# khanhha/temporal_inverse_kinematics

Measured on AMD Instinct MI355X. Metric: IK frames/sec (COCO-17->SMPLx pose), higher is better.
Workload: dtype f32 via bf16x3 (x = 3 bf16 planes, 6 MFMA products, fp32 accumulate; fp32 exponent range); 1 GPU; ST-GCN IK forward, batch=1024x64-frame x COCO-17 windows per GPU -> (B,4,66) SMPL-X pose; global_batch=1024, window_frames=64, out_frames=4, parallelism=single

## Files before the change

### include/tik.h

```cpp
#ifndef TIK_H
#define TIK_H

#include <stdint.h>

#ifdef __cplusplus
extern "C" {
#endif

#define TIK_OK 0
#define TIK_E_INVALID (-1)
#define TIK_E_HIP (-2)
#define TIK_E_MISSING (-3)
#define TIK_E_NOMEM (-4)

typedef struct tik_model* tik_model_t;
typedef struct tik_fk* tik_fk_t;

typedef struct {
    const char* name;
    const float* data;
    int ndim;
    int64_t shape[4];
} tik_tensor;

const char* tik_last_error(void);
const char* tik_version(void);
int tik_debug_check_guards(void);
int tik_debug_alloc_fill(void);
int tik_debug_checksums(char* buf, int len);

int tik_model_create(const tik_tensor* tensors, int n_tensors, tik_model_t* out);
int tik_model_destroy(tik_model_t m);
int tik_model_out_frames(tik_model_t m, int T);
int tik_model_reserve(tik_model_t m, int N, int T);
int tik_ik_forward(tik_model_t m, const float* x, int N, int T, float* poses, void* stream);
int tik_backbone_forward(tik_model_t m, const float* x, int N, int T, float* feat, void* stream);

#define TIK_PREC_F32 0
#define TIK_PREC_BF16X3 2
int tik_model_set_precision(tik_model_t m, int prec);
int tik_model_get_precision(tik_model_t m);

int tik_model_profile(tik_model_t m, int max_launches);
int tik_model_profile_count(tik_model_t m);
int tik_model_profile_read(tik_model_t m, int i, char* label, int label_len, float* ms, double* flops,
                           double* bytes);

typedef struct tik_block* tik_block_t;
int tik_block_create(const tik_tensor* tensors, int n_tensors, int in_channels, int out_channels,
                     int stride, int residual, const float* A_eff_host, int V, tik_block_t* out);
int tik_block_destroy(tik_block_t b);
int tik_stgcn_block_fwd(tik_block_t b, const float* x, int N, int T, float* out, void* stream);
int tik_block_set_precision(tik_block_t b, int prec);

int tik_gconv_fwd(const float* x, int N, int Cin, int T, int V, const float* A, int K,
                  const float* W, const float* b, int Cout, int t_kernel, int t_stride,
                  int t_padding, int t_dilation, float* out, void* stream);

int tik_aa_to_rotmat(const float* aa, int n, float* R, void* stream);

int tik_window_gather(const float* seq, int F, int V, int idx0, int n_idx, int h, int root_a,
                      int root_b, int relative, float* windows, void* stream);

int tik_moveai_to_coco(const float* joints, int F, int J, const int* map17_host, float* out, void* stream);

typedef struct tik_stream* tik_stream_t;
int tik_stream_create(tik_model_t model, int win_size, int use_graph, tik_stream_t* out);
int tik_stream_destroy(tik_stream_t s);
int tik_stream_reset(tik_stream_t s);
int tik_stream_push(tik_stream_t s, const float* frame_host, float* pose_host);
int tik_stream_path(tik_stream_t s);
int tik_debug_stream_trace(tik_stream_t s, long long* out, int cap);
int tik_debug_stream_inject_error(tik_stream_t s);
int tik_debug_stream_set_count(tik_stream_t s, int count);

int tik_rotate_root_z(float* poses, int F, int ld, double angle, void* stream);
int tik_train_windows(const float* joints, int n_joints, const float* poses, int pose_ld, const int* item_start,
                      const int* item_len, const int* item_idx, const int* item_uid, int B, int h,
                      const int* coco_map, const float* sigma, int relative, int add_noise, unsigned long long seed,
                      float* windows, float* target, void* stream);

typedef struct tik_trainer* tik_trainer_t;
// ... 35 lines not shown
```

### temporal_inverse_kinematics_amd/_lib.py

```python
from __future__ import annotations

import ctypes
import os
from typing import Dict, Iterable, Tuple

import numpy as np
import torch

LIB_PATH = os.environ.get("TIK_LIB") or os.path.join(os.path.dirname(os.path.abspath(__file__)), "libtik.so")

TIK_OK, TIK_E_INVALID, TIK_E_HIP, TIK_E_MISSING, TIK_E_NOMEM = 0, -1, -2, -3, -4


class TikTensor(ctypes.Structure):
    _fields_ = [("name", ctypes.c_char_p), ("data", ctypes.POINTER(ctypes.c_float)),
                ("ndim", ctypes.c_int), ("shape", ctypes.c_int64 * 4)]


_P = ctypes.c_void_p
_I = ctypes.c_int
_F = ctypes.POINTER(ctypes.c_float)

SIGNATURES: Dict[str, Tuple[object, Tuple]] = {
    "tik_last_error": (ctypes.c_char_p, ()),
    "tik_version": (ctypes.c_char_p, ()),
    "tik_debug_check_guards": (_I, ()),
    "tik_debug_alloc_fill": (_I, ()),
    "tik_debug_checksums": (_I, (ctypes.c_char_p, _I)),
    "tik_model_create": (_I, (ctypes.POINTER(TikTensor), _I, ctypes.POINTER(_P))),
    "tik_model_destroy": (_I, (_P,)),
    "tik_model_out_frames": (_I, (_P, _I)),
    "tik_model_reserve": (_I, (_P, _I, _I)),
    "tik_ik_forward": (_I, (_P, _P, _I, _I, _P, _P)),
    "tik_backbone_forward": (_I, (_P, _P, _I, _I, _P, _P)),
    "tik_model_set_precision": (_I, (_P, _I)),
    "tik_model_get_precision": (_I, (_P,)),
    "tik_block_set_precision": (_I, (_P, _I)),
    "tik_fk_set_precision": (_I, (_P, _I)),
    "tik_model_profile": (_I, (_P, _I)),
    "tik_model_profile_count": (_I, (_P,)),
    "tik_model_profile_read": (_I, (_P, _I, ctypes.c_char_p, _I, ctypes.POINTER(ctypes.c_float),
                                    ctypes.POINTER(ctypes.c_double), ctypes.POINTER(ctypes.c_double))),
    "tik_block_create": (_I, (ctypes.POINTER(TikTensor), _I, _I, _I, _I, _I, _F, _I, ctypes.POINTER(_P))),
    "tik_block_destroy": (_I, (_P,)),
    "tik_stgcn_block_fwd": (_I, (_P, _P, _I, _I, _P, _P)),
    "tik_gconv_fwd": (_I, (_P, _I, _I, _I, _I, _P, _I, _P, _P, _I, _I, _I, _I, _I, _P, _P)),
    "tik_aa_to_rotmat": (_I, (_P, _I, _P, _P)),
    "tik_window_gather": (_I, (_P, _I, _I, _I, _I, _I, _I, _I, _I, _P, _P)),
    "tik_moveai_to_coco": (_I, (_P, _I, _I, ctypes.POINTER(ctypes.c_int), _P, _P)),
    "tik_stream_create": (_I, (_P, _I, _I, ctypes.POINTER(_P))),
    "tik_stream_destroy": (_I, (_P,)),
    "tik_stream_reset": (_I, (_P,)),
    "tik_stream_push": (_I, (_P, _F, _F)),
    "tik_stream_path": (_I, (_P,)),
    "tik_rotate_root_z": (_I, (_P, _I, _I, ctypes.c_double, _P)),
    "tik_train_windows": (_I, (_P, _I, _P, _I, _P, _P, _P, _P, _I, _I, _P, _P, _I, _I, ctypes.c_ulonglong, _P, _P, _P)),
    "tik_debug_stream_trace": (_I, (_P, ctypes.POINTER(ctypes.c_longlong), _I)),
    "tik_debug_stream_inject_error": (_I, (_P,)),
    "tik_debug_stream_set_count": (_I, (_P, _I)),
    "tik_fk_create": (_I, (ctypes.POINTER(TikTensor), _I, _I, ctypes.POINTER(_P))),
    "tik_fk_destroy": (_I, (_P,)),
    "tik_fk_num_joints": (_I, (_P,)),
    "tik_fk_num_verts": (_I, (_P,)),
    "tik_fk_reserve": (_I, (_P, _I)),
    "tik_fk_forward": (_I, (_P, _P, _P, _P, _P, _I, _P, _P, _P)),
    "tik_fk_joints": (_I, (_P, _P, _P, _P, _P, _I, ctypes.POINTER(_I), _I, _P, _P)),
    "tik_fk_workspace_bytes": (ctypes.c_longlong, (_P,)),
    "tik_fk_profile": (_I, (_P, _I)),
    "tik_fk_profile_count": (_I, (_P,)),
    "tik_fk_profile_read": (_I, (_P, _I, ctypes.c_char_p, _I, ctypes.POINTER(ctypes.c_float),
                                 ctypes.POINTER(ctypes.c_double), ctypes.POINTER(ctypes.c_double))),
    "tik_trainer_create": (_I, (ctypes.POINTER(TikTensor), _I, ctypes.c_float, ctypes.POINTER(_P))),
    "tik_trainer_destroy": (_I, (_P,)),
    "tik_trainer_step": (_I, (_P, _P, _I, _I, _P, _P, ctypes.c_ulonglong, _P, _P)),
    "tik_trainer_out_frames": (_I, (_P, _I)),
    "tik_trainer_count": (_I, (_P,)),
    "tik_trainer_tensor": (_I, (_P, _I, ctypes.c_char_p, _I, ctypes.POINTER(ctypes.c_int64), ctypes.POINTER(_I),
                                ctypes.POINTER(_I))),
    "tik_trainer_read": (_I, (_P, _I, _I, _P, _P)),
    "tik_trainer_steps": (ctypes.c_longlong, (_P,)),
    "tik_trainer_debug": (_I, (_P, _I, _I, _P, ctypes.c_longlong, _P)),
# ... 85 lines not shown
```

### temporal_inverse_kinematics_amd/csrc/debug.cpp

```cpp
#include <hip/hip_runtime.h>

#include <algorithm>
#include <map>
#include <mutex>

#include "misc.h"
#include "model.h"

namespace tik_host {
std::atomic<int> g_alloc_fill{-1};
thread_local Profiler* g_prof = nullptr;

bool guard_mode() {
    static const bool on = getenv("TIK_GUARD") && getenv("TIK_GUARD")[0] == '1';
    return on;
}
static std::mutex g_guard_mu;
static std::map<void*, size_t> g_guard_bufs;
void guard_register(void* base, size_t bytes) {
    std::lock_guard<std::mutex> l(g_guard_mu);
    g_guard_bufs[base] = bytes;
}
void guard_unregister(void* base) {
    std::lock_guard<std::mutex> l(g_guard_mu);
// ... 97 lines not shown
}
using namespace tik_host;

extern "C" {

int tik_debug_checksums(char* buf, int len) {
    if (!checksum_mode()) return fail(TIK_E_INVALID, "TIK_CHECKSUM is not set");
    const int n = (int)g_cks.size();
    if (buf && len > 0) {
        strncpy(buf, g_cks.c_str(), len - 1);
        buf[len - 1] = 0;
    }
    g_cks.clear();
    return n;
}

int tik_debug_check_guards(void) {
    if (!guard_mode()) return fail(TIK_E_INVALID, "TIK_GUARD=1 is not set");
    HIP_TRY(hipDeviceSynchronize());
    std::lock_guard<std::mutex> l(g_guard_mu);
    std::vector<unsigned char> h(GUARD_BYTES);
    int bad = 0;
    std::string rep;
    for (const auto& kv : g_guard_bufs) {
        const char* base = static_cast<const char*>(kv.first);
        for (int side = 0; side < 2; ++side) {
            const char* gp = side == 0 ? base : base + GUARD_BYTES + kv.second;
            HIP_TRY(hipMemcpy(h.data(), gp, GUARD_BYTES, hipMemcpyDeviceToHost));
            size_t first = GUARD_BYTES, last = 0, cnt = 0;
            bool clean = true;
            for (size_t i = 0; i < GUARD_BYTES && clean; i += 8) {
                unsigned long long w;
                memcpy(&w, h.data() + i, 8);
                clean = w == 0xA5A5A5A5A5A5A5A5ull;
            }
            for (size_t i = 0; i < GUARD_BYTES && !clean; ++i)
                if (h[i] != 0xA5) { first = std::min(first, i); last = i; ++cnt; }
            if (cnt) {
                ++bad;
                char b[256];
                snprintf(b, sizeof(b), "[buf %p payload %zu B: %s guard, %zu bytes changed at +%zu..+%zu] ", (const void*)(base + GUARD_BYTES),
                         kv.second, side == 0 ? "front" : "back", cnt, first, last);
                rep += b;
                HIP_TRY(hipMemset(const_cast<char*>(gp), 0xA5, GUARD_BYTES));
            }
        }
    }
    g_err = rep;
    return bad;
}

int tik_debug_alloc_fill(void) { return g_alloc_fill.load(); }

}
```

### temporal_inverse_kinematics_amd/csrc/forward.cpp

```cpp
#include <hip/hip_runtime.h>

#include <algorithm>

#include "misc.h"
#include "model.h"
#include "xtws.h"

using namespace tik_host;

namespace tik_host {

static tik::Seg mkseg(const float* src, const float* w, const SplitW3& s3, int cin, int ld, int kt, int stride, int pad,
                      int tin, int ldw) {
    tik::Seg s{src, w, cin, ld, kt, stride, pad, tin, ldw};
    s.cin8 = s3.cin8; s.ldw8 = s3.ldw8;
    for (int i = 0; i < 3; ++i) s.wb[i] = s3.p[i].p;
    return s;
}

int Layer::forward(const float* x, int ld, int N, int tin, float* z, float* out, hipStream_t st, int prec,
                   float* part) const {
    const int to = tout(tin, stride);
    tik::CgemmArgs g{};
    g.M = N * tin * V; g.Nc = cout; g.V = V; g.tout = tin;
    g.seg[0] = mkseg(x, wg.p, s3g, cinp, ld, 1, 1, 0, tin, cinp);
    g.nseg = 1;
    g.bias = bias2.p; g.out = z; g.ldo = cout; g.amix = amix.p; g.act = tik::ACT_RELU;
    g.mix_sparse = mix_sparse ? 1 : 0;
    const double px_in = (double)N * tin * V, px_out = (double)N * to * V;
    {
        const std::string lab = "G272x64.L" + std::to_string(index);
        ProfScope p(lab.c_str(), gcn_work(px_in, cin, cout, V), st);
        HIP_TRY(tik::launch_cgemm(g, tik::CFG_G272x64, st, prec));
    }

    tik::CgemmArgs t{};
    t.M = N * to * V; t.Nc = cout; t.V = V; t.tout = to;
    t.seg[0] = mkseg(z, wt.p, s3t, cout, cout, TK, stride, 1, tin, TK * cout);
    t.nseg = 1;
    if (res == RES_CONV) {
        t.seg[1] = mkseg(x, wr.p, s3r, cinp, ld, 1, stride, 0, tin, cinp);
        t.nseg = 2;
    } else if (res == RES_IDEN) {
        t.resid = x; t.ldr = ld;
    }
    t.bias = biasT.p; t.out = out; t.ldo = cout; t.act = tik::ACT_RELU;
    const bool big = cout >= 128;
    const int cfg = big ? tik::CFG_T128x128 : (prec == tik::PREC_F32 ? tik::CFG_T256x64 : tik::CFG_T128x64);
    const std::string lab = std::string(big ? "T128x128.L" : (cfg == tik::CFG_T256x64 ? "T256x64.L" : "T128x64.L")) +
                            std::to_string(index);
    if (part) {
        t.ksplit = tik::splitk_for(t, cfg == tik::CFG_T256x64 ? 256 : 128, big ? 128 : 64,
                                   prec == tik::PREC_F32 ? 16 : 32, 64);
        t.partial = part;
    }
    ProfScope p(lab.c_str(), tcn_work(px_in, px_out, cin, cout, res), st);
    HIP_TRY(tik::launch_cgemm(t, cfg, st, prec));
    return TIK_OK;
}

int Layer::spatial_x(const float* x, int ld, int N, int tin, float* z, hipStream_t st, int ncu, const RawInput* raw) const {
    const long long rin = (long long)N * tin * V;
    if (raw) {
        ProfScope p("G0f_raw.L0", gcn_work((double)rin, cin, cout, V, GCN_RAW0), st);
        HIP_TRY(tik::launch_gcn0_f32(raw->kp, (int)rin, V, cin, raw->bn_sc, raw->bn_sh, wg.p, cinp, bias2.p, amix.p, mix_sparse ? 1 : 0,
                                     cout, z, cout, raw->xb4, st));
    } else if (xgw_path()) {
        tik::XGraphArgs g{};
        g.nframes = N * tin; g.x = x; g.ldx = ld; g.cin = cin; g.cout = cout; g.wp = xgw.p;
        g.bias2 = bias2.p; g.amix = amix.p; g.mix_sparse = mix_sparse ? 1 : 0; g.out = z; g.ldo = cout;
        g.nts = 1; g.trash = xtrash;
        const std::string lab = "XGW.L" + std::to_string(index);
        ProfScope p(lab.c_str(), gcn_work((double)rin, cin, cout, V), st);
        p.out(z, (size_t)rin * cout * 4);
        HIP_TRY(launch_xgraph_traced(g, ncu, st, lab.c_str()));
    } else {
        tik::XArgs g{};
        g.M = (int)rin; g.Nc = cout; g.V = V; g.tout = tin;
        g.seg[0] = tik::XSeg{x, ld, cin, 1, 1, 0, tin, rin};
        g.nseg = 1; g.wp = xg.p; g.ksteps = xg_ks;
        g.bias = bias2.p; g.amix = amix.p; g.mix_sparse = mix_sparse ? 1 : 0; g.out = z; g.ldo = cout; g.act = tik::ACT_RELU;
        g.nw = 4; g.nts = 1;
        const std::string lab = std::string(xg_bn == 128 ? "XG128.L" : "XG64.L") + std::to_string(index);
        ProfScope p(lab.c_str(), gcn_work((double)rin, cin, cout, V), st);
        p.out(z, (size_t)rin * cout * 4);
        HIP_TRY(launch_xgemm_traced(g, xg_bn, tik::EPI_GRAPH, st, lab.c_str()));
    }
    return TIK_OK;
}

int Layer::temporal_x(const float* x, int ld, int N, int tin, const float* z, float* out, hipStream_t st, int ncu,
                      const RawInput* raw, const FusedNext* fg) const {
    const int to = tout(tin, stride);
    const long long rin = (long long)N * tin * V, rout = (long long)N * to * V;
    const double px_in = (double)rin, px_out = (double)rout;
    if (xtws_path(raw != nullptr, ld, tin)) {
        tik::XTConvArgs c{};
        c.M = (int)rout; c.T = tin; c.z = z; c.ldz = cout; c.x = x; c.ldx = ld; c.wp = xtw.p; c.bias = biasT.p;
        c.out = out; c.ldo = cout; c.nts = 1; c.trash = xtrash;
        Work w = tcn_work(px_in, px_out, cin, cout, RES_IDEN);
        if (fg) {
            const Layer& gn = *fg->layer;
            c.wg = gn.xgw.p; c.bias2 = gn.bias2.p; c.amix = gn.amix.p; c.mix_sparse = gn.mix_sparse ? 1 : 0;
            c.zout = fg->zn; c.ldzo = gn.cout;
            w = w + gcn_work(px_out, gn.cin, gn.cout, V, GCN_FUSED);
        }
        const std::string lab = (fg ? "XTWG.L" : "XTW.L") + std::to_string(index);
        ProfScope p(lab.c_str(), w, st);
        p.out(out, (size_t)rout * cout * 4);
        HIP_TRY(tik::launch_xtws(c, ncu, st));
        return TIK_OK;
    }
    tik::XArgs t{};
    t.M = (int)rout; t.Nc = cout; t.V = V; t.tout = to;
    t.seg[0] = tik::XSeg{z, cout, cout, TK, stride, 1, tin, rin};
    t.nseg = 1;
    if (raw) {
        t.rx = raw->xb4; t.rxc = cin; t.rw = wr0.p;
    } else if (res == RES_CONV) {
        t.seg[1] = tik::XSeg{x, ld, cin, 1, stride, 0, tin, rin};
        t.nseg = 2;
    } else if (res == RES_IDEN) {
        t.idn = tik::XSeg{x, ld, cin, 1, 1, 0, to, rin};
    }
    t.wp = xt.p; t.ksteps = tik::xgemm_ksteps(t);
    if (tik::xgemm_kmain(t) != xt_ks) return fail(TIK_E_INVALID, "layer %d: xgemm K steps %d != packed %d", index, tik::xgemm_kmain(t), xt_ks);
    t.bias = biasT.p; t.out = out; t.ldo = cout; t.act = tik::ACT_RELU;
    t.nw = 4; t.epi_lds = 1; t.idn_epi = 1; t.nts = 1;
// ... 264 lines not shown
```

### temporal_inverse_kinematics_amd/csrc/model.cpp

```cpp
#include <hip/hip_runtime.h>

#include <algorithm>
#include <memory>

#include "model.h"
#include "online.h"

using namespace tik_host;

namespace tik_host {

int Layer::pack(const FoldedBlock& f) {
    cin = f.cin; cinp = f.cinp; cout = f.cout; stride = f.stride; res = f.res; V = f.V; mix_sparse = f.mix_sparse;
    int rc;
    if ((rc = wg.upload(f.wg)) || (rc = bias2.upload(f.bias2)) || (rc = amix.upload(f.amix)) || (rc = wt.upload(f.wt)) ||
        (rc = biasT.upload(f.biasT)) || (rc = s3g.build(f.wg, cout, 1, cinp, cinp)) ||
        (rc = s3t.build(f.wt, cout, TK, cout, TK * cout)))
        return rc;
    if (res == RES_CONV && ((rc = wr.upload(f.wr)) || (rc = s3r.build(f.wr, cout, 1, cinp, cinp)))) return rc;
    if ((rc = wr0.upload(f.wr0))) return rc;
    const int bn = cout >= 128 ? 128 : 64;
    if (cin % 32 == 0) {
        const tik::XPackSeg g{f.wg.data(), cinp, 1, cin};
        if ((rc = xg.upload(tik::xgemm_pack(&g, 1, cout, bn)))) return rc;
        xg_bn = bn; xg_ks = cin / 32;
    }
    if (cout % 32 == 0) {
        tik::XPackSeg t[2] = {{f.wt.data(), TK * cout, TK, cout}, {f.wr.data(), cinp, 1, cin}};
        const int ns = (res == RES_CONV && cin % 32 == 0) ? 2 : 1;
        if ((rc = xt.upload(tik::xgemm_pack(t, ns, cout, bn)))) return rc;
        xt_bn = bn; xt_ks = TK * cout / 32 + (ns == 2 ? cin / 32 : 0);
    }
    if (cout == 128 && cin == 128 && stride == 1 && res == RES_IDEN)
        if ((rc = xtw.upload(tik::xblock_pack_weights(f.wt.data(), cout, TK * cout, TK, cout)))) return rc;
    if ((cout == 128 || cout == 256) && (cin == 64 || cin == 128 || cin == 256))
        if ((rc = xgw.upload(tik::xblock_pack_weights(f.wg.data(), cout, cinp, 1, cin)))) return rc;
    if (cout == 64 && stride == 1) {
        if ((rc = xbt.upload(tik::xblock_pack_weights(f.wt.data(), cout, TK * cout, TK, cout)))) return rc;
        if (cin == 64 && (rc = xbg.upload(tik::xblock_pack_weights(f.wg.data(), cout, cinp, 1, cin)))) return rc;
    }
    return TIK_OK;
}

static void apply_env(tik_model* md) {
    if (const char* e = getenv("TIK_X_CHUNK")) md->x_chunk_max = atoi(e);
    if (const char* e = getenv("TIK_XBLK")) md->xblk = e[0] != '0';
    int dev = 0, ncu = 0;
    if (hipGetDevice(&dev) == hipSuccess && hipDeviceGetAttribute(&ncu, hipDeviceAttributeMultiprocessorCount, dev) == hipSuccess && ncu > 0)
        md->ncu = ncu;
    for (auto& L : md->layers) {
        if (const char* w = getenv("TIK_XGW")) L.xgwon = (atoi(w) >> L.index) & 1;
        if (const char* w = getenv("TIK_XTWS")) L.xtwson = (atoi(w) >> L.index) & 1;
        if (const char* w = getenv("TIK_XFG")) L.xfgon = (atoi(w) >> L.index) & 1;
        L.xtrash = reinterpret_cast<float*>(md->trash.p);
    }
    if (const char* e = getenv("TIK_SPLIT")) md->split = e[0] != '0';
}

int model_reserve_ws(tik_model* m, Workspace& w, int N, int T) {
    const size_t V = m->V;
    size_t zmax = 0, amax = 0;
    int t = T;
    for (const Layer& L : m->layers) {
        zmax = std::max(zmax, (size_t)N * t * V * L.cout);
        t = Layer::tout(t, L.stride);
        amax = std::max(amax, (size_t)N * t * V * L.cout);
    }
    if (m->use_xblk()) zmax = std::max(zmax, (size_t)N * T * V * XB0_P3_FLOATS);
    size_t z2max = 0;
    t = T;
    for (size_t l = 0; l + 1 < m->layers.size(); ++l) {
        const Layer& L = m->layers[l];
        t = Layer::tout(t, L.stride);
        if (L.index > 0 && L.stride == 1 && L.fuses_gcn_of(m->layers[l + 1])) z2max = std::max(z2max, (size_t)N * t * V * m->layers[l + 1].cout);
    }
    t = T;
    for (const Layer& L : m->layers) t = Layer::tout(t, L.stride);
    int rc;
    if (z2max && (rc = w.z2.reserve(z2max))) return rc;
    if ((rc = w.xb.reserve((size_t)N * T * V * 4)) || (rc = w.z.reserve(zmax)) ||
        (rc = w.a0.reserve(amax)) || (rc = w.a1.reserve(amax)) || (rc = w.hid.reserve((size_t)N * t * m->hidden)) ||
        (rc = w.part.reserve(std::max((size_t)384 * 128 * 128, (size_t)8 * N * t * m->hidden))))
        return rc;
    return TIK_OK;
}

void model_retain(tik_model* m) { m->refs.fetch_add(1); }
int model_pose_dim(const tik_model* m) { return m->pose_dim; }
void model_release(tik_model* m) {
    if (m->refs.fetch_sub(1) == 1) delete m;
}

int model_online_fill(tik_model* m, tik::OnlineArgs& a) {
    static_assert((int)tik::ONR_ZERO == RES_ZERO && (int)tik::ONR_IDEN == RES_IDEN && (int)tik::ONR_CONV == RES_CONV, "");
    const int nl = (int)m->layers.size();
    if (m->V != 17 || m->C0 != 3 || nl > tik::ONL_MAXL) return fail(TIK_E_INVALID, "online kernel: V=17, 3 input channels, <= %d layers", tik::ONL_MAXL);
    if (m->pose_dim <= 0) return fail(TIK_E_INVALID, "online kernel: backbone-only handle (no pose_regressor weights)");
    a.nl = nl;
    for (int l = 0; l < nl; ++l) {
        const Layer& L = m->layers[l];
        if (L.cout % 16 || L.cout > tik::ONL_MAXC || L.cinp > tik::ONL_MAXC || (l > 0 && L.cinp != L.cin))
            return fail(TIK_E_INVALID, "online kernel: layer %d channels %d -> %d", l, L.cin, L.cout);
        tik::OnlineLayer& o = a.L[l];
        o.cin = L.cin; o.cinp = L.cinp; o.cout = L.cout; o.stride = L.stride; o.res = L.res;
// ... 88 lines not shown
```

### temporal_inverse_kinematics_amd/csrc/model.h

```cpp
#pragma once
#include <atomic>
#include <string>
#include <vector>

#include "cgemm.h"
#include "common.h"
#include "xblock.h"
#include "xgemm.h"
#include "xgraph.h"

namespace tik_host {

struct Work {
    double flops = 0, bytes = 0;
    Work operator+(const Work& o) const { return Work{flops + o.flops, bytes + o.bytes}; }
};
enum GcnIo {
    GCN_LAYER = 0,
    GCN_RAW0 = 1,
    GCN_FUSED = 2,
};
inline Work gcn_work(double px, int cin, int cout, int V, GcnIo io = GCN_LAYER) {
    const double x = io == GCN_FUSED ? 0.0 : px * cin;
    const double w = io == GCN_RAW0 ? 0.0 : (double)cout * cin + (double)V * (V + cout);
    return Work{2.0 * px * cin * cout + 2.0 * V * px * cout, 4.0 * (x + px * cout + w)};
}
constexpr int RES_RAW0 = 3;
inline Work tcn_work(double px_in, double px_out, int cin, int cout, int res) {
    Work w{2.0 * px_out * TK * cout * cout, 4.0 * (px_in * cout + px_out * cout + (double)TK * cout * cout)};
    if (res == RES_CONV || res == RES_RAW0) w.flops += 2.0 * px_out * cin * cout;
    if (res == RES_CONV) w.bytes += 4.0 * (px_out * cin + (double)cin * cout);
    if (res == RES_RAW0) w.bytes += 4.0 * px_out * 4;
    if (res == RES_IDEN) w.bytes += 4.0 * px_out * cout;
    return w;
}

extern thread_local Profiler* g_prof;

struct ProfScope {
    int i;
    hipStream_t st;
    const char* lab;
    const void* op = nullptr;
    size_t obytes = 0;
    void out(const void* p, size_t bytes) { op = p; obytes = bytes; }
    ProfScope(const char* label, Work w, hipStream_t s) : st(s), lab(label) {
        i = g_prof ? g_prof->begin(label, w.flops, w.bytes, s) : -1;
    }
    ~ProfScope();
};

hipError_t launch_xgemm_traced(tik::XArgs a, int bn, int epi, hipStream_t st, const char* label);
hipError_t launch_xgraph_traced(tik::XGraphArgs a, int ncu, hipStream_t st, const char* label);
hipError_t launch_xblock_traced(tik::XBlkArgs a, bool raw, int ncu, hipStream_t st, const char* label);

struct Layer;
struct RawInput {
    const float *kp, *bn_sc, *bn_sh;
    float* xb4;
};
struct FusedNext {
    const Layer* layer;
    float* zn;
};

struct Layer {
    int cin = 0, cinp = 0, cout = 0, stride = 1, res = RES_IDEN, V = 17, index = 0;
    bool mix_sparse = false;
    DevBuf wg, bias2, amix, wt, wr, biasT;
    SplitW3 s3g, s3t, s3r;
    DevBuf wr0;
    DevHBuf xg, xt;
    int xg_bn = 0, xt_bn = 0, xg_ks = 0, xt_ks = 0;
    DevHBuf xtw;
    DevHBuf xgw;
    DevHBuf xbg, xbt;
    int xgwon = 1;
    int xtwson = 1;
    int xfgon = 1;
    float* xtrash = nullptr;

    int pack(const FoldedBlock& f);

    static int tout(int tin, int s) { return (tin - 1) / s + 1; }

    bool x_ok() const { return xt.p && (xg.p || (index == 0 && wr0.p)); }
    bool xgw_path() const { return xgwon && xgw.p; }
    bool xtws_path(bool raw, int ld, int tin) const {
        return xtwson && xtw.p && !raw && res == RES_IDEN && stride == 1 && ld >= cout && ld % 4 == 0 && tin % 8 == 0;
    }
    bool fuses_gcn_of(const Layer& nx) const {
        return xfgon && xtw.p && nx.xgw_path() && nx.cin == cout && cout == 128 && nx.cout == 128;
    }
    bool xpt_path() const { return xt_bn == 64 && cout % xt_bn == 0; }

    int forward(const float* x, int ld, int N, int tin, float* z, float* out, hipStream_t st, int prec,
                float* part = nullptr) const;
    int spatial_x(const float* x, int ld, int N, int tin, float* z, hipStream_t st, int ncu,
                  const RawInput* raw) const;
    int temporal_x(const float* x, int ld, int N, int tin, const float* z, float* out, hipStream_t st, int ncu,
                   const RawInput* raw, const FusedNext* fg) const;
};

}

struct tik_model {
    int V = 17, C0 = 3, feat = 0, hidden = 0, pose_dim = 0;
    std::vector<tik_host::Layer> layers;
    tik_host::DevBuf bn_sc, bn_sh;
    tik_host::DevBuf w0, b0, w3, b3;
    tik_host::SplitW3 s30, s33;
    tik_host::DevHBuf xh0;
    static constexpr int XHEAD_KS = 4;
    int prec = 2;
    static constexpr int MAXSPLIT = 2;
    tik_host::Workspace ws[MAXSPLIT];
    hipStream_t aux[MAXSPLIT - 1] = {};
    hipEvent_t ev_fork = nullptr, ev_join[MAXSPLIT - 1] = {};
    bool split = true;
    std::atomic<int> refs{1};
    ~tik_model() {
        if (ev_fork) (void)hipEventDestroy(ev_fork);
        for (auto e : ev_join) if (e) (void)hipEventDestroy(e);
        for (auto a : aux) if (a) (void)hipStreamDestroy(a);
    }
    int x_chunk_max = 0;
    bool xblk = true;
    int ncu = 256;
    tik_host::DevHBuf trash;
    tik_host::Profiler prof;
// ... 31 lines not shown
```

### temporal_inverse_kinematics_amd/csrc/xgraph.h

```cpp
#pragma once
#include <hip/hip_runtime.h>

namespace tik {

struct XGraphArgs {
    int nframes;
    const float* x;
    int ldx;
    int cin, cout;
    const unsigned short* wp;
    const float* bias2;
    const float* amix;
    int mix_sparse;
    float* out;
    int ldo;
    int nts;
    float* trash;
    int tune;
    unsigned long long* trace;
};

bool xgraph_ok(const XGraphArgs& a);
hipError_t launch_xgraph(const XGraphArgs& a, int ncu, hipStream_t st);

}
```

### temporal_inverse_kinematics_amd/csrc/xgraph.hip

```cpp
#include <algorithm>
#include <type_traits>

#include "xgemm_dev.h"
#include "xgraph.h"

namespace tik {

namespace xg {
constexpr int V = 17, FR = 16, PX = FR * V;
constexpr int NU = PX * 8;
constexpr int NLD = (NU + 511) / 512;
constexpr int PROWB = 3 * 32 * 2;
constexpr int PBYTES = PX * PROWB;
}

__device__ __forceinline__ int xg_unit(int R, int p, int u) { return R * xg::PROWB + ((p * 4 + (u ^ ((R >> 1) & 3))) << 4); }

__device__ f32x4 tik_llvm_raw_buffer_load_v4f32(i32x4 rsrc, int voffset, int soffset, int aux)
    __asm("llvm.amdgcn.raw.buffer.load.v4f32");

typedef __bf16 xbf16x4 __attribute__((ext_vector_type(4)));

#ifdef TIK_XTUNE
#define XG_OFF(bit) (a.tune & (bit))
#else
#define XG_OFF(bit) false
#endif

template <int NK, int NP>
__global__ __launch_bounds__(512, 1) void xgraph_kernel(XGraphArgs a) {
    using namespace xg;
    constexpr int D = NK <= 4 ? 2 : 1;
    constexpr int B2MAX = V * 256 * 4;
    __shared__ __attribute__((aligned(16))) unsigned char smem[2 * PBYTES + B2MAX];
    float* const b2s = reinterpret_cast<float*>(smem + 2 * PBYTES);
    auto pimg = [&](int s) __attribute__((always_inline)) { return smem + (s & 1) * PBYTES; };

    int tid = threadIdx.x, lane = tid & 63;
    const int wave = __builtin_amdgcn_readfirstlane(tid >> 6);
    const int QO = a.nframes, M = QO * V;
    constexpr int npass = NP;
    const int nfg = (QO + FR - 1) / FR;
    const int ntiles = nfg * npass;
    int t_begin, t_end;
    {
        const int nwg = gridDim.x, bid = blockIdx.x;
        const int per = nwg >> 3, rem = nwg & 7, x = bid & 7, k = bid >> 3;
        const int s = x < rem ? x * (per + 1) + k : rem * (per + 1) + (x - rem) * per + k;
        t_begin = (int)((long long)s * ntiles / nwg);
        t_end = (int)((long long)(s + 1) * ntiles / nwg);
    }
    if (t_begin >= t_end) return;
    const int total = (t_end - t_begin) * NK;
    auto tile_fg = [&](int t) __attribute__((always_inline)) { return t / npass; };
    auto tile_pass = [&](int t) __attribute__((always_inline)) { return t - (t / npass) * npass; };

    for (int i = tid; i < V * a.cout; i += 512) b2s[i] = a.bias2[i];
    float amv[5];
#pragma unroll
    for (int k = 0; k < 5; ++k) amv[k] = 64 * k + lane < V * V ? a.amix[64 * k + lane] : 0.f;

    const i32x4 rX = buf_rsrc(a.x, (unsigned)((long long)M * a.ldx * 4));
    f32x4 rb[D][NLD];
    auto load_unit = [&](int s, f32x4 (&r)[NLD], int i) __attribute__((always_inline)) {
        const int t = t_begin + s / NK, kb = s - (s / NK) * NK;
        const int q0 = tile_fg(t) * FR;
        const bool live = s < total;
        const int U = 512 * i + tid, m = U >> 3, u = U & 7;
        const int q = q0 + m / V;
        const unsigned off = live && U < NU && q < QO && !XG_OFF(1) ? (unsigned)(((long long)q0 * V + m) * a.ldx * 4 + kb * 128 + u * 16) : DMA_OOB;
        r[i] = tik_llvm_raw_buffer_load_v4f32(rX, (int)off, 0, 2);
    };
    auto load = [&](int s, f32x4 (&r)[NLD]) __attribute__((always_inline)) {
#pragma unroll
        for (int i = 0; i < NLD; ++i) load_unit(s, r, i);
    };
    auto split_unit = [&](int s, const f32x4 (&r)[NLD], int i) __attribute__((always_inline)) {
        unsigned char* P = pimg(s);
        const int U = 512 * i + tid;
        if (i + 1 < NLD || U < NU) {
            const int m = U >> 3, u = U & 7;
            const int R = 16 * (m % V) + m / V;
            xbf16x4 p0, p1, p2;
#pragma unroll
            for (int e = 0; e < 4; ++e) {
                const float x = r[i][e];
                const __bf16 b0 = (__bf16)x;
                const float r1 = x - (float)b0;
                const __bf16 b1 = (__bf16)r1;
                p0[e] = b0;
                p1[e] = b1;
                p2[e] = (__bf16)(r1 - (float)b1);
            }
            const int h = (u & 1) * 8;
            *reinterpret_cast<xbf16x4*>(P + xg_unit(R, 0, u >> 1) + h) = p0;
            *reinterpret_cast<xbf16x4*>(P + xg_unit(R, 1, u >> 1) + h) = p1;
            *reinterpret_cast<xbf16x4*>(P + xg_unit(R, 2, u >> 1) + h) = p2;
        }
    };
    auto split = [&](int s, const f32x4 (&r)[NLD]) __attribute__((always_inline)) {
#pragma unroll
        for (int i = 0; i < NLD; ++i) split_unit(s, r, i);
    };

    xbf16x8 w[NK][3];
    auto load_wk = [&](int pass, int kb) __attribute__((always_inline)) {
        const int cg = pass * 8 + wave;
#pragma unroll
        for (int p = 0; p < 3; ++p)
            w[kb][p] = *reinterpret_cast<const xbf16x8*>(a.wp + ((((size_t)cg * NK + kb) * 3 + p) * 64 + lane) * 8);
    };
    auto load_w = [&](int pass) __attribute__((always_inline)) {
#pragma unroll
        for (int kb = 0; kb < NK; ++kb) load_wk(pass, kb);
    };

    load(0, rb[0]);
    load_w(tile_pass(t_begin));
    split(0, rb[0]);
#pragma unroll
    for (int d = 1; d <= D; ++d) load(d, rb[d % D]);

    f32x4 acc[V];
#pragma unroll
    for (int j = 0; j < V; ++j) acc[j] = f32x4{0.f, 0.f, 0.f, 0.f};

#ifdef TIK_XTRACE
    const bool tr = a.trace != nullptr && (wave == 0 || wave == 4);
#else
    constexpr bool tr = false;
#endif
    unsigned long long ph_[6] = {0, 0, 0, 0, 0, 0}, tlast = 0, tstart = 0;
    auto stamp = [&](int i) __attribute__((always_inline)) {
        if (tr) {
            const unsigned long long t = __builtin_amdgcn_s_memtime();
            if (i >= 0) ph_[i] += t - tlast;
            else tstart = t;
            tlast = t;
        }
    };
    stamp(-1);

    auto step = [&](int s, int t, int pass, auto KBc) __attribute__((always_inline)) {
        constexpr int kb = decltype(KBc)::value;
        constexpr int nb = (kb + 1) % D;
        asm volatile("" : "+v"(tid), "+v"(lane));
        const int g = lane >> 4, f = lane & 15;
        lds_barrier();
        stamp(0);
        const unsigned char* P = pimg(s);
        constexpr int XPF = 2;
        xbf16x8 xb[XPF + 1][3];
        auto rd = [&](int j, xbf16x8 (&d)[3]) __attribute__((always_inline)) {
#pragma unroll
            for (int p = 0; p < 3; ++p) d[p] = *reinterpret_cast<const xbf16x8*>(P + xg_unit(16 * j + f, p, g));
        };
        auto mfma_j = [&](int j) __attribute__((always_inline)) {
            if (j + XPF < V) rd(j + XPF, xb[(j + XPF) % (XPF + 1)]);
            __builtin_amdgcn_sched_barrier(0);
            if (XG_OFF(4)) return;
            const xbf16x8(&x)[3] = xb[j % (XPF + 1)];
            acc[j] = __builtin_amdgcn_mfma_f32_16x16x32_bf16(w[kb][0], x[2], acc[j], 0, 0, 0);
            acc[j] = __builtin_amdgcn_mfma_f32_16x16x32_bf16(w[kb][1], x[1], acc[j], 0, 0, 0);
            acc[j] = __builtin_amdgcn_mfma_f32_16x16x32_bf16(w[kb][2], x[0], acc[j], 0, 0, 0);
            acc[j] = __builtin_amdgcn_mfma_f32_16x16x32_bf16(w[kb][0], x[1], acc[j], 0, 0, 0);
            acc[j] = __builtin_amdgcn_mfma_f32_16x16x32_bf16(w[kb][1], x[0], acc[j], 0, 0, 0);
            acc[j] = __builtin_amdgcn_mfma_f32_16x16x32_bf16(w[kb][0], x[0], acc[j], 0, 0, 0);
            __builtin_amdgcn_sched_barrier(0);
        };
#pragma unroll
        for (int j = 0; j < XPF; ++j) rd(j, xb[j]);
        if constexpr (NP == 2) {
#pragma unroll
            for (int j = 0; j < V; ++j) {
                mfma_j(j);
                if (j % 3 == 1 && j / 3 < NLD) {
                    const int i = j / 3;
                    if (!XG_OFF(2)) split_unit(s + 1, rb[nb], i);
                    load_unit(s + 1 + D, rb[nb], i);
                    asm volatile("" ::: "memory");
                    __builtin_amdgcn_sched_barrier(0);
                }
                if (j == 3) {
                    stamp(1);
                    stamp(2);
                    stamp(3);
                }
            }
        } else {
#pragma unroll
            for (int j = 0; j < 4; ++j) mfma_j(j);
            stamp(1);
            if (!XG_OFF(2)) split(s + 1, rb[nb]);
            stamp(2);
            load(s + 1 + D, rb[nb]);
            stamp(3);
#pragma unroll
            for (int j = 4; j < V; ++j) mfma_j(j);
        }
        stamp(4);
        if constexpr (NP == 2) load_wk(tile_pass(t + 1), kb);
        if constexpr (kb == NK - 1) {
            const int co = pass * 128 + 16 * wave + 4 * g;
            const int q = tile_fg(t) * FR + f;
            auto mix_all = [&](auto sparse) __attribute__((always_inline)) {
                constexpr bool SP = decltype(sparse)::value;
#pragma unroll
                for (int wj = 0; wj < V; ++wj) {
                    f32x4 z = *reinterpret_cast<const f32x4*>(b2s + wj * a.cout + co);
#pragma unroll
                    for (int v = 0; v < V; ++v)
                        if (XG_OFF(16)) {
                            if (v == wj) z += acc[v];
                        } else if (!SP || ((coco_hop2_mask3(wj) >> v) & 1u)) {
                            const float av = __builtin_bit_cast(
                                float, __builtin_amdgcn_readlane(__builtin_bit_cast(int, amv[(v * V + wj) / 64]), (v * V + wj) % 64));
                            z += av * acc[v];
                        }
#pragma unroll
                    for (int e = 0; e < 4; ++e) z[e] = z[e] > 0.f ? z[e] : 0.f;
                    float* o = q < QO ? a.out + ((size_t)q * V + wj) * a.ldo + co : a.trash;
                    if (!XG_OFF(8)) xst4(o, z, a.nts);
                }
            };
            if (a.mix_sparse) mix_all(std::true_type{});
            else mix_all(std::false_type{});
#pragma unroll
            for (int j = 0; j < V; ++j) acc[j] = f32x4{0.f, 0.f, 0.f, 0.f};
            stamp(5);
        }
    };
    for (int t = t_begin; t < t_end; ++t) {
        const int s0 = (t - t_begin) * NK, pass = tile_pass(t);
        step(s0, t, pass, std::integral_constant<int, 0>{});
        step(s0 + 1, t, pass, std::integral_constant<int, 1>{});
        if constexpr (NK > 2) {
            step(s0 + 2, t, pass, std::integral_constant<int, 2>{});
            step(s0 + 3, t, pass, std::integral_constant<int, 3>{});
        }
        if constexpr (NK > 4) {
            step(s0 + 4, t, pass, std::integral_constant<int, 4>{});
            step(s0 + 5, t, pass, std::integral_constant<int, 5>{});
            step(s0 + 6, t, pass, std::integral_constant<int, 6>{});
            step(s0 + 7, t, pass, std::integral_constant<int, 7>{});
        }
    }
    asm volatile("s_waitcnt vmcnt(0)" ::: "memory");
#ifdef TIK_XTRACE
    if (tr && lane == 0) {
        unsigned long long* o = a.trace + 16 * (size_t)blockIdx.x + (wave == 4 ? 8 : 0);
#pragma unroll
        for (int i = 0; i < 6; ++i) o[i] = ph_[i];
        o[6] = (unsigned long long)total;
        o[7] = tlast - tstart;
    }
#endif
}

bool xgraph_ok(const XGraphArgs& a) {
    return (a.cin == 64 || a.cin == 128 || a.cin == 256) && (a.cout == 128 || a.cout == 256) && a.ldx % 4 == 0 &&
           a.ldx >= a.cin && a.ldo % 4 == 0 && a.ldo >= a.cout;
}

hipError_t launch_xgraph(const XGraphArgs& a, int ncu, hipStream_t st) {
    if (a.nframes <= 0) return hipSuccess;
    if (!xgraph_ok(a) || !a.x || !a.wp || !a.bias2 || !a.amix || !a.out || !a.trash || ncu <= 0) return hipErrorInvalidValue;
    const long long row_bytes = 17LL * a.ldx * 4;
    const int chunk = (int)std::min<long long>(a.nframes, ((1LL << 31) - 1) / row_bytes / xg::FR * xg::FR);
    if (chunk <= 0) return hipErrorInvalidValue;
    (void)hipGetLastError();
    for (int q0 = 0; q0 < a.nframes; q0 += chunk) {
        XGraphArgs c = a;
        c.nframes = std::min(chunk, a.nframes - q0);
        c.x = a.x + (size_t)q0 * 17 * a.ldx;
        c.out = a.out + (size_t)q0 * 17 * a.ldo;
        const int ntiles = ((c.nframes + xg::FR - 1) / xg::FR) * (a.cout / 128);
        const int grid = std::min(ntiles, ncu);
        const bool two = a.cout == 256;
        if (a.cin == 64) hipLaunchKernelGGL((two ? xgraph_kernel<2, 2> : xgraph_kernel<2, 1>), dim3(grid), dim3(512), 0, st, c);
        else if (a.cin == 128) hipLaunchKernelGGL((two ? xgraph_kernel<4, 2> : xgraph_kernel<4, 1>), dim3(grid), dim3(512), 0, st, c);
        else hipLaunchKernelGGL((two ? xgraph_kernel<8, 2> : xgraph_kernel<8, 1>), dim3(grid), dim3(512), 0, st, c);
        const hipError_t e = hipGetLastError();
        if (e != hipSuccess) return e;
    }
    return hipSuccess;
}

}
```

Baseline: 348,900 IK frames/s.

## Hoist xgraph load offsets, per-tile buffer descriptors, and decouple weight prefetch depth

```diff
diff --git a/include/tik.h b/include/tik.h
--- a/include/tik.h
+++ b/include/tik.h
@@ -28,6 +28,7 @@
 int tik_debug_check_guards(void);
 int tik_debug_alloc_fill(void);
 int tik_debug_checksums(char* buf, int len);
+int tik_debug_xgraph_runs(int nframes, int cout, int ncu, int cap, int* runs, int max_runs);
 
 int tik_model_create(const tik_tensor* tensors, int n_tensors, tik_model_t* out);
 int tik_model_destroy(tik_model_t m);
diff --git a/temporal_inverse_kinematics_amd/_lib.py b/temporal_inverse_kinematics_amd/_lib.py
--- a/temporal_inverse_kinematics_amd/_lib.py
+++ b/temporal_inverse_kinematics_amd/_lib.py
@@ -27,6 +27,7 @@
     "tik_debug_check_guards": (_I, ()),
     "tik_debug_alloc_fill": (_I, ()),
     "tik_debug_checksums": (_I, (ctypes.c_char_p, _I)),
+    "tik_debug_xgraph_runs": (_I, (_I, _I, _I, _I, ctypes.POINTER(_I), _I)),
     "tik_model_create": (_I, (ctypes.POINTER(TikTensor), _I, ctypes.POINTER(_P))),
     "tik_model_destroy": (_I, (_P,)),
     "tik_model_out_frames": (_I, (_P, _I)),
diff --git a/temporal_inverse_kinematics_amd/csrc/debug.cpp b/temporal_inverse_kinematics_amd/csrc/debug.cpp
--- a/temporal_inverse_kinematics_amd/csrc/debug.cpp
+++ b/temporal_inverse_kinematics_amd/csrc/debug.cpp
@@ -173,4 +173,12 @@
 
 int tik_debug_alloc_fill(void) { return g_alloc_fill.load(); }
 
+int tik_debug_xgraph_runs(int nframes, int cout, int ncu, int cap, int* runs, int max_runs) {
+    if (nframes <= 0 || (cout != 128 && cout != 256) || ncu <= 0) return fail(TIK_E_INVALID, "tik_debug_xgraph_runs: bad arguments");
+    const int ntiles = tik::xgraph_tiles(nframes, cout);
+    const int grid = std::min(ntiles, tik::xgraph_grid_cap(ncu, cap));
+    for (int b = 0; runs && b < grid && b < max_runs; ++b) tik::xgraph_run(ntiles, grid, b, runs[2 * b], runs[2 * b + 1]);
+    return grid;
 }
+
+}
diff --git a/temporal_inverse_kinematics_amd/csrc/forward.cpp b/temporal_inverse_kinematics_amd/csrc/forward.cpp
--- a/temporal_inverse_kinematics_amd/csrc/forward.cpp
+++ b/temporal_inverse_kinematics_amd/csrc/forward.cpp
@@ -73,7 +73,7 @@
         const std::string lab = "XGW.L" + std::to_string(index);
         ProfScope p(lab.c_str(), gcn_work((double)rin, cin, cout, V), st);
         p.out(z, (size_t)rin * cout * 4);
-        HIP_TRY(launch_xgraph_traced(g, ncu, st, lab.c_str()));
+        HIP_TRY(launch_xgraph_traced(g, tik::xgraph_grid_cap(ncu, xgw_grid), st, lab.c_str()));
     } else {
         tik::XArgs g{};
         g.M = (int)rin; g.Nc = cout; g.V = V; g.tout = tin;
diff --git a/temporal_inverse_kinematics_amd/csrc/model.cpp b/temporal_inverse_kinematics_amd/csrc/model.cpp
--- a/temporal_inverse_kinematics_amd/csrc/model.cpp
+++ b/temporal_inverse_kinematics_amd/csrc/model.cpp
@@ -50,6 +50,7 @@
         md->ncu = ncu;
     for (auto& L : md->layers) {
         if (const char* w = getenv("TIK_XGW")) L.xgwon = (atoi(w) >> L.index) & 1;
+        if (const char* w = getenv("TIK_XGW_GRID")) L.xgw_grid = atoi(w);
         if (const char* w = getenv("TIK_XTWS")) L.xtwson = (atoi(w) >> L.index) & 1;
         if (const char* w = getenv("TIK_XFG")) L.xfgon = (atoi(w) >> L.index) & 1;
         L.xtrash = reinterpret_cast<float*>(md->trash.p);
diff --git a/temporal_inverse_kinematics_amd/csrc/model.h b/temporal_inverse_kinematics_amd/csrc/model.h
--- a/temporal_inverse_kinematics_amd/csrc/model.h
+++ b/temporal_inverse_kinematics_amd/csrc/model.h
@@ -76,6 +76,7 @@
     DevHBuf xgw;
     DevHBuf xbg, xbt;
     int xgwon = 1;
+    int xgw_grid = 0;
     int xtwson = 1;
     int xfgon = 1;
     float* xtrash = nullptr;
diff --git a/temporal_inverse_kinematics_amd/csrc/xgraph.h b/temporal_inverse_kinematics_amd/csrc/xgraph.h
--- a/temporal_inverse_kinematics_amd/csrc/xgraph.h
+++ b/temporal_inverse_kinematics_amd/csrc/xgraph.h
@@ -21,6 +21,14 @@
 };
 
 bool xgraph_ok(const XGraphArgs& a);
+inline int xgraph_tiles(int nframes, int cout) { return ((nframes + 15) / 16) * (cout / 128); }
+inline int xgraph_grid_cap(int ncu, int cap) { return cap > 0 && cap < ncu ? cap : ncu; }
+__host__ __device__ inline void xgraph_run(int ntiles, int nwg, int bid, int& t_begin, int& t_end) {
+    const int per = nwg >> 3, rem = nwg & 7, x = bid & 7, k = bid >> 3;
+    const int s = x < rem ? x * (per + 1) + k : rem * (per + 1) + (x - rem) * per + k;
+    t_begin = (int)((long long)s * ntiles / nwg);
+    t_end = (int)((long long)(s + 1) * ntiles / nwg);
+}
 hipError_t launch_xgraph(const XGraphArgs& a, int ncu, hipStream_t st);
 
 }
diff --git a/temporal_inverse_kinematics_amd/csrc/xgraph.hip b/temporal_inverse_kinematics_amd/csrc/xgraph.hip
--- a/temporal_inverse_kinematics_amd/csrc/xgraph.hip
+++ b/temporal_inverse_kinematics_amd/csrc/xgraph.hip
@@ -28,13 +28,22 @@
 #endif
 
 template <int NK, int NP>
+struct XgCfg {
+    static constexpr int D = NP == 2 ? 2 : NK <= 4 ? 2 : 1;
+    static constexpr int R = NP == 2 ? 2 : NK;
+    static constexpr bool HOIST = !(NK == 8 && NP == 1);
+    static_assert(NK % D == 0 && NK % R == 0 && R >= D, "D and R divide NK; R >= D");
+};
+
+template <int NK, int NP>
 __global__ __launch_bounds__(512, 1) void xgraph_kernel(XGraphArgs a) {
     using namespace xg;
-    constexpr int D = NK <= 4 ? 2 : 1;
+    constexpr int D = XgCfg<NK, NP>::D;
+    constexpr int R = XgCfg<NK, NP>::R;
+    constexpr bool HOIST = XgCfg<NK, NP>::HOIST;
     constexpr int B2MAX = V * 256 * 4;
     __shared__ __attribute__((aligned(16))) unsigned char smem[2 * PBYTES + B2MAX];
     float* const b2s = reinterpret_cast<float*>(smem + 2 * PBYTES);
-    auto pimg = [&](int s) __attribute__((always_inline)) { return smem + (s & 1) * PBYTES; };
 
     int tid = threadIdx.x, lane = tid & 63;
     const int wave = __builtin_amdgcn_readfirstlane(tid >> 6);
@@ -43,15 +52,8 @@
     const int nfg = (QO + FR - 1) / FR;
     const int ntiles = nfg * npass;
     int t_begin, t_end;
-    {
-        const int nwg = gridDim.x, bid = blockIdx.x;
-        const int per = nwg >> 3, rem = nwg & 7, x = bid & 7, k = bid >> 3;
-        const int s = x < rem ? x * (per + 1) + k : rem * (per + 1) + (x - rem) * per + k;
-        t_begin = (int)((long long)s * ntiles / nwg);
-        t_end = (int)((long long)(s + 1) * ntiles / nwg);
-    }
+    xgraph_run(ntiles, gridDim.x, blockIdx.x, t_begin, t_end);
     if (t_begin >= t_end) return;
-    const int total = (t_end - t_begin) * NK;
     auto tile_fg = [&](int t) __attribute__((always_inline)) { return t / npass; };
     auto tile_pass = [&](int t) __attribute__((always_inline)) { return t - (t / npass) * npass; };
 
@@ -60,27 +62,44 @@
 #pragma unroll
     for (int k = 0; k < 5; ++k) amv[k] = 64 * k + lane < V * V ? a.amix[64 * k + lane] : 0.f;
 
-    const i32x4 rX = buf_rsrc(a.x, (unsigned)((long long)M * a.ldx * 4));
+    auto unit_voff = [&](int i) __attribute__((always_inline)) {
+        const int U = 512 * i + tid, m = U >> 3, u = U & 7;
+        return U < NU ? (unsigned)((m * a.ldx + 4 * u) * 4) : DMA_OOB;
+    };
+    auto unit_lds = [&](int i) __attribute__((always_inline)) {
+        const int U = 512 * i + tid, m = U >> 3, u = U & 7;
+        return xg_unit(16 * (m % V) + m / V, 0, u >> 1) + (u & 1) * 8;
+    };
+    unsigned voff_[NLD];
+    int lds_[NLD];
+    if constexpr (HOIST) {
+#pragma unroll
+        for (int i = 0; i < NLD; ++i) {
+            voff_[i] = unit_voff(i);
+            lds_[i] = unit_lds(i);
+            asm volatile("" : "+v"(voff_[i]), "+v"(lds_[i]));
+        }
+    }
+    auto voff = [&](int i) __attribute__((always_inline)) { return HOIST ? voff_[i] : unit_voff(i); };
+    auto ldsa = [&](int i) __attribute__((always_inline)) { return HOIST ? lds_[i] : unit_lds(i); };
+    const long long xbytes = (long long)M * a.ldx * 4, gbytes = (long long)FR * V * a.ldx * 4;
+    auto rsrc_tile = [&](int t) __attribute__((always_inline)) {
+        const long long o = tile_fg(t) * gbytes;
+        return buf_rsrc(reinterpret_cast<const unsigned char*>(a.x) + o, t < t_end && !XG_OFF(1) ? (unsigned)(xbytes - o) : 0u);
+    };
     f32x4 rb[D][NLD];
-    auto load_unit = [&](int s, f32x4 (&r)[NLD], int i) __attribute__((always_inline)) {
-        const int t = t_begin + s / NK, kb = s - (s / NK) * NK;
-        const int q0 = tile_fg(t) * FR;
-        const bool live = s < total;
-        const int U = 512 * i + tid, m = U >> 3, u = U & 7;
-        const int q = q0 + m / V;
-        const unsigned off = live && U < NU && q < QO && !XG_OFF(1) ? (unsigned)(((long long)q0 * V + m) * a.ldx * 4 + kb * 128 + u * 16) : DMA_OOB;
-        r[i] = tik_llvm_raw_buffer_load_v4f32(rX, (int)off, 0, 2);
-    };
-    auto load = [&](int s, f32x4 (&r)[NLD]) __attribute__((always_inline)) {
-#pragma unroll
-        for (int i = 0; i < NLD; ++i) load_unit(s, r, i);
-    };
-    auto split_unit = [&](int s, const f32x4 (&r)[NLD], int i) __attribute__((always_inline)) {
-        unsigned char* P = pimg(s);
-        const int U = 512 * i + tid;
-        if (i + 1 < NLD || U < NU) {
-            const int m = U >> 3, u = U & 7;
-            const int R = 16 * (m % V) + m / V;
+    auto load_unit = [&](const i32x4& rs, auto KBc, f32x4 (&r)[NLD], int i) __attribute__((always_inline)) {
+        constexpr int kb = decltype(KBc)::value;
+        r[i] = tik_llvm_raw_buffer_load_v4f32(rs, (int)(voff(i) + kb * 128), 0, 2);
+    };
+    auto load = [&](const i32x4& rs, auto KBc, f32x4 (&r)[NLD]) __attribute__((always_inline)) {
+#pragma unroll
+        for (int i = 0; i < NLD; ++i) load_unit(rs, KBc, r, i);
+    };
+    auto split_unit = [&](auto IMGc, const f32x4 (&r)[NLD], int i) __attribute__((always_inline)) {
+        constexpr int img = decltype(IMGc)::value;
+        static_assert((NU - 512 * (NLD - 1)) % 64 == 0, "the last unit round ends on a wave");
+        if (i + 1 < NLD || wave < (NU - 512 * (NLD - 1)) / 64) {
             xbf16x4 p0, p1, p2;
 #pragma unroll
             for (int e = 0; e < 4; ++e) {
@@ -92,34 +111,36 @@
                 p1[e] = b1;
                 p2[e] = (__bf16)(r1 - (float)b1);
             }
-            const int h = (u & 1) * 8;
-            *reinterpret_cast<xbf16x4*>(P + xg_unit(R, 0, u >> 1) + h) = p0;
-            *reinterpret_cast<xbf16x4*>(P + xg_unit(R, 1, u >> 1) + h) = p1;
-            *reinterpret_cast<xbf16x4*>(P + xg_unit(R, 2, u >> 1) + h) = p2;
-        }
-    };
-    auto split = [&](int s, const f32x4 (&r)[NLD]) __attribute__((always_inline)) {
-#pragma unroll
-        for (int i = 0; i < NLD; ++i) split_unit(s, r, i);
-    };
-
-    xbf16x8 w[NK][3];
+            unsigned char* P = smem + ldsa(i);
+            *reinterpret_cast<xbf16x4*>(P + img * PBYTES) = p0;
+            *reinterpret_cast<xbf16x4*>(P + img * PBYTES + 64) = p1;
+            *reinterpret_cast<xbf16x4*>(P + img * PBYTES + 128) = p2;
+        }
+    };
+    auto split = [&](auto IMGc, const f32x4 (&r)[NLD]) __attribute__((always_inline)) {
+#pragma unroll
+        for (int i = 0; i < NLD; ++i) split_unit(IMGc, r, i);
+    };
+
+    xbf16x8 w[R][3];
     auto load_wk = [&](int pass, int kb) __attribute__((always_inline)) {
         const int cg = pass * 8 + wave;
 #pragma unroll
         for (int p = 0; p < 3; ++p)
-            w[kb][p] = *reinterpret_cast<const xbf16x8*>(a.wp + ((((size_t)cg * NK + kb) * 3 + p) * 64 + lane) * 8);
-    };
-    auto load_w = [&](int pass) __attribute__((always_inline)) {
-#pragma unroll
-        for (int kb = 0; kb < NK; ++kb) load_wk(pass, kb);
-    };
-
-    load(0, rb[0]);
-    load_w(tile_pass(t_begin));
-    split(0, rb[0]);
-#pragma unroll
-    for (int d = 1; d <= D; ++d) load(d, rb[d % D]);
+            w[kb % R][p] = *reinterpret_cast<const xbf16x8*>(a.wp + ((((size_t)cg * NK + kb) * 3 + p) * 64 + lane) * 8);
+    };
+
+    auto pro_load = [&](auto Dc) __attribute__((always_inline)) {
+        constexpr int d = decltype(Dc)::value;
+        load(rsrc_tile(t_begin + d / NK), std::integral_constant<int, d % NK>{}, rb[d % D]);
+    };
+    pro_load(std::integral_constant<int, 0>{});
+#pragma unroll
+    for (int kb = 0; kb < R; ++kb) load_wk(tile_pass(t_begin), kb);
+    split(std::integral_constant<int, 0>{}, rb[0]);
+    pro_load(std::integral_constant<int, 1>{});
+    if constexpr (D == 2) pro_load(std::integral_constant<int, 2>{});
+    static_assert(D == 1 || D == 2, "prologue unrolled by hand");
 
     f32x4 acc[V];
 #pragma unroll
@@ -141,14 +162,17 @@
     };
     stamp(-1);
 
-    auto step = [&](int s, int t, int pass, auto KBc) __attribute__((always_inline)) {
+    auto step = [&](int t, int pass, auto KBc) __attribute__((always_inline)) {
         constexpr int kb = decltype(KBc)::value;
         constexpr int nb = (kb + 1) % D;
+        using NImg = std::integral_constant<int, (kb + 1) & 1>;
+        using NKb = std::integral_constant<int, (kb + 1 + D) % NK>;
+        const i32x4 rN = rsrc_tile(t + (kb + 1 + D) / NK);
         asm volatile("" : "+v"(tid), "+v"(lane));
         const int g = lane >> 4, f = lane & 15;
         lds_barrier();
         stamp(0);
-        const unsigned char* P = pimg(s);
+        const unsigned char* P = smem + (kb & 1) * PBYTES;
         constexpr int XPF = 2;
         xbf16x8 xb[XPF + 1][3];
         auto rd = [&](int j, xbf16x8 (&d)[3]) __attribute__((always_inline)) {
@@ -160,12 +184,13 @@
             __builtin_amdgcn_sched_barrier(0);
             if (XG_OFF(4)) return;
             const xbf16x8(&x)[3] = xb[j % (XPF + 1)];
-            acc[j] = __builtin_amdgcn_mfma_f32_16x16x32_bf16(w[kb][0], x[2], acc[j], 0, 0, 0);
-            acc[j] = __builtin_amdgcn_mfma_f32_16x16x32_bf16(w[kb][1], x[1], acc[j], 0, 0, 0);
-            acc[j] = __builtin_amdgcn_mfma_f32_16x16x32_bf16(w[kb][2], x[0], acc[j], 0, 0, 0);
-            acc[j] = __builtin_amdgcn_mfma_f32_16x16x32_bf16(w[kb][0], x[1], acc[j], 0, 0, 0);
-            acc[j] = __builtin_amdgcn_mfma_f32_16x16x32_bf16(w[kb][1], x[0], acc[j], 0, 0, 0);
-            acc[j] = __builtin_amdgcn_mfma_f32_16x16x32_bf16(w[kb][0], x[0], acc[j], 0, 0, 0);
+            const xbf16x8(&wk)[3] = w[kb % R];
+            acc[j] = __builtin_amdgcn_mfma_f32_16x16x32_bf16(wk[0], x[2], acc[j], 0, 0, 0);
+            acc[j] = __builtin_amdgcn_mfma_f32_16x16x32_bf16(wk[1], x[1], acc[j], 0, 0, 0);
+            acc[j] = __builtin_amdgcn_mfma_f32_16x16x32_bf16(wk[2], x[0], acc[j], 0, 0, 0);
+            acc[j] = __builtin_amdgcn_mfma_f32_16x16x32_bf16(wk[0], x[1], acc[j], 0, 0, 0);
+            acc[j] = __builtin_amdgcn_mfma_f32_16x16x32_bf16(wk[1], x[0], acc[j], 0, 0, 0);
+            acc[j] = __builtin_amdgcn_mfma_f32_16x16x32_bf16(wk[0], x[0], acc[j], 0, 0, 0);
             __builtin_amdgcn_sched_barrier(0);
         };
 #pragma unroll
@@ -176,8 +201,8 @@
                 mfma_j(j);
                 if (j % 3 == 1 && j / 3 < NLD) {
                     const int i = j / 3;
-                    if (!XG_OFF(2)) split_unit(s + 1, rb[nb], i);
-                    load_unit(s + 1 + D, rb[nb], i);
+                    if (!XG_OFF(2)) split_unit(NImg{}, rb[nb], i);
+                    load_unit(rN, NKb{}, rb[nb], i);
                     asm volatile("" ::: "memory");
                     __builtin_amdgcn_sched_barrier(0);
                 }
@@ -191,15 +216,18 @@
 #pragma unroll
             for (int j = 0; j < 4; ++j) mfma_j(j);
             stamp(1);
-            if (!XG_OFF(2)) split(s + 1, rb[nb]);
+            if (!XG_OFF(2)) split(NImg{}, rb[nb]);
             stamp(2);
-            load(s + 1 + D, rb[nb]);
+            load(rN, NKb{}, rb[nb]);
             stamp(3);
 #pragma unroll
             for (int j = 4; j < V; ++j) mfma_j(j);
         }
         stamp(4);
-        if constexpr (NP == 2) load_wk(tile_pass(t + 1), kb);
+        if constexpr (NP == 2) {
+            if constexpr (kb + R < NK) load_wk(pass, kb + R);
+            else load_wk(tile_pass(t + 1), kb + R - NK);
+        }
         if constexpr (kb == NK - 1) {
             const int co = pass * 128 + 16 * wave + 4 * g;
             const int q = tile_fg(t) * FR + f;
@@ -231,18 +259,18 @@
         }
     };
     for (int t = t_begin; t < t_end; ++t) {
-        const int s0 = (t - t_begin) * NK, pass = tile_pass(t);
-        step(s0, t, pass, std::integral_constant<int, 0>{});
-        step(s0 + 1, t, pass, std::integral_constant<int, 1>{});
+        const int pass = tile_pass(t);
+        step(t, pass, std::integral_constant<int, 0>{});
+        step(t, pass, std::integral_constant<int, 1>{});
         if constexpr (NK > 2) {
-            step(s0 + 2, t, pass, std::integral_constant<int, 2>{});
-            step(s0 + 3, t, pass, std::integral_constant<int, 3>{});
+            step(t, pass, std::integral_constant<int, 2>{});
+            step(t, pass, std::integral_constant<int, 3>{});
         }
         if constexpr (NK > 4) {
-            step(s0 + 4, t, pass, std::integral_constant<int, 4>{});
-            step(s0 + 5, t, pass, std::integral_constant<int, 5>{});
-            step(s0 + 6, t, pass, std::integral_constant<int, 6>{});
-            step(s0 + 7, t, pass, std::integral_constant<int, 7>{});
+            step(t, pass, std::integral_constant<int, 4>{});
+            step(t, pass, std::integral_constant<int, 5>{});
+            step(t, pass, std::integral_constant<int, 6>{});
+            step(t, pass, std::integral_constant<int, 7>{});
         }
     }
     asm volatile("s_waitcnt vmcnt(0)" ::: "memory");
@@ -251,7 +279,7 @@
         unsigned long long* o = a.trace + 16 * (size_t)blockIdx.x + (wave == 4 ? 8 : 0);
 #pragma unroll
         for (int i = 0; i < 6; ++i) o[i] = ph_[i];
-        o[6] = (unsigned long long)total;
+        o[6] = (unsigned long long)(t_end - t_begin) * NK;
         o[7] = tlast - tstart;
     }
 #endif
@@ -274,8 +302,7 @@
         c.nframes = std::min(chunk, a.nframes - q0);
         c.x = a.x + (size_t)q0 * 17 * a.ldx;
         c.out = a.out + (size_t)q0 * 17 * a.ldo;
-        const int ntiles = ((c.nframes + xg::FR - 1) / xg::FR) * (a.cout / 128);
-        const int grid = std::min(ntiles, ncu);
+        const int grid = std::min(xgraph_tiles(c.nframes, a.cout), ncu);
         const bool two = a.cout == 256;
         if (a.cin == 64) hipLaunchKernelGGL((two ? xgraph_kernel<2, 2> : xgraph_kernel<2, 1>), dim3(grid), dim3(512), 0, st, c);
         else if (a.cin == 128) hipLaunchKernelGGL((two ? xgraph_kernel<4, 2> : xgraph_kernel<4, 1>), dim3(grid), dim3(512), 0, st, c);
```

Result: no change. 352,100 IK frames/s, median of 6 (+0.9%).
